# ChaissonLab/LRA

Measured on AMD Instinct MI355X. Metric: aligned Gbp/s, 30 kb ONT vs GRCh38 (MapRead_lowacc end to end incl. SAM text), per job, higher is better.
Workload: dtype int32

## Files before the change

### include/lra_hip.h

```cpp
#ifndef LRA_HIP_H_
#define LRA_HIP_H_
#include <stddef.h>
#include <stdint.h>

#ifdef __cplusplus
extern "C" {
#endif

typedef struct lra_ctx lra_ctx;

#define LRA_OK 0
#define LRA_ERR_INVALID (-1)
#define LRA_ERR_HIP (-2)
#define LRA_ERR_NOMEM (-3)

#define LRA_ST_OOB_SLOT 1
#define LRA_ST_NO_TERMINATION 2
#define LRA_ST_RANGE 4
#define LRA_ST_CAPACITY 8
#define LRA_ST_REJECTED 16
#define LRA_ST_UNSUPPORTED 32
#define LRA_ST_DEFERRED 64

int lra_ctx_create(int device_id, lra_ctx** out);
// ... 230 lines not shown
                           int mismatch, int indel, int max_freq, lra_refine_space_result* out);
int lra_refine_space_batch_mf(lra_ctx* ctx, int n, const char* d_qseq, const uint64_t* d_q_off, const int32_t* d_q_len, const char* d_tseq,
                              const uint64_t* d_t_off, const int32_t* d_t_len, const uint32_t* d_t_span, const int32_t* d_K, const int32_t* d_W,
                              const int32_t* d_diag, const uint32_t* d_q_add, const uint32_t* d_t_add, const uint32_t* d_flip_len, int match,
                              int mismatch, int indel, const int32_t* d_max_freq, lra_refine_space_result* out);

typedef struct lra_btwn_opts { int32_t K, W, refineSpaceDist; float anchorstoosparse; int32_t match, mismatch, indel, max_freq; } lra_btwn_opts;
typedef struct lra_btwn_result {
  uint64_t n_frags, n_matches, n_problems, n_pairs; uint32_t n_rounds;
  const uint64_t* d_match_off; const uint32_t* d_match_q; const uint32_t* d_match_t;
  const uint32_t* d_box; const float* d_eff; const uint8_t* d_refinespace;
} lra_btwn_result;
int lra_refine_btwn_splitchain_batch(lra_ctx* ctx, const lra_chain_result* chains, const lra_split_result* split, const lra_refined_result* refined,
                                     const uint64_t* d_read_off, const char* d_strands, uint64_t rc_base, const char* d_genome,
                                     const uint64_t* h_chrom_pos, int n_chrom, const lra_btwn_opts* opts, lra_btwn_result* out);

typedef struct lra_merge_result {
  uint64_t n_slots, n_groups, n_anchors;
  const uint64_t* d_slot_group_off;
  const uint64_t* d_cluster_base;
  const uint32_t* d_group_slot; const uint32_t* d_group_first; const uint32_t* d_group_last;
  const uint64_t* d_anchor_off;
  const uint32_t* d_count;
  const uint32_t* d_q; const uint32_t* d_t; const int32_t* d_len;
  const uint32_t* d_box; const int32_t* d_strand; const int32_t* d_chrom;
  const uint64_t* d_iota;
} lra_merge_result;
int lra_trim_anchor_pairs_batch(lra_ctx* ctx, uint64_t n_lists, const uint64_t* d_off, uint64_t n_anchors, uint32_t* d_q, uint32_t* d_t, int32_t* d_len);
int lra_trim_overlapped_anchors_batch(lra_ctx* ctx, uint64_t n_clusters, const uint64_t* d_off, uint64_t n_anchors, const int32_t* d_strand,
                                      uint32_t* d_q, uint32_t* d_t, int32_t* d_len);
// ... 437 lines not shown
```

### lra_amd/_lib.py

```python
import ctypes as C
import os

HERE = os.path.dirname(os.path.abspath(__file__))
_LIB = None
ABI_VERSION = 9


class LraError(RuntimeError):
    pass


def library_path():
    return os.path.join(HERE, "liblra_hip.so")


_u64p = C.POINTER(C.c_uint64)
_i32p = C.POINTER(C.c_int32)
_vp = C.c_void_p
SYMBOLS = {
    "lra_abi_version": (C.c_int, []),
    "lra_ctx_create": (C.c_int, [C.c_int, C.POINTER(_vp)]),
    "lra_ctx_destroy": (None, [_vp]),
    "lra_ctx_release_buffers": (C.c_int, [_vp, _u64p]),
    "lra_ctx_set_stream": (C.c_int, [_vp, _vp]),
# ... 73 lines not shown
    "lra_global_chain_batch": (C.c_int, [_vp, C.c_uint64, _vp, C.c_uint64, _vp, _vp, _vp, _vp, _vp, _vp]),
    "lra_split_chains_highacc_batch": (C.c_int, [_vp, C.c_uint64, _vp, C.c_uint64, _vp, _vp, _vp, _vp, _vp, C.c_int, _vp]),
    "lra_split_chains_batch": (C.c_int, [_vp, _vp, _vp, C.c_int, C.c_int, C.c_int, _vp]),
    "lra_format_sam": (C.c_int, [_vp, C.c_int, C.c_int, C.c_int, C.c_char_p, _vp, C.c_uint64, _vp]),
    "lra_format_sam_simple": (C.c_int, [_vp, C.c_int, C.c_char_p, _vp, C.c_uint64, _vp]),
    "lra_format_paf": (C.c_int, [_vp, C.c_int, _vp, C.c_uint64, _vp]),
    "lra_format_bed": (C.c_int, [_vp, _vp, C.c_uint64, _vp]),
    "lra_refine_space_batch": (C.c_int, [_vp, C.c_int] + [_vp] * 13 + [C.c_int] * 4 + [_vp]),
    "lra_refine_space_batch_mf": (C.c_int, [_vp, C.c_int] + [_vp] * 13 + [C.c_int] * 3 + [_vp, _vp]),
    "lra_between_anchors_batch": (C.c_int, [_vp, C.c_int] + [_vp] * 8 + [C.c_int] * 5 + [_vp]),
    "lra_refine_breakpoint_batch": (C.c_int, [_vp, C.c_int] + [_vp] * 16),
    "lra_sparse_dp_boxes_batch": (C.c_int, [_vp, C.c_int, _vp, _vp, _vp, _vp, _vp, _vp, _vp, _vp, _vp, _vp, _vp, _vp]),
    "lra_split_clusters_batch": (C.c_int, [_vp, C.c_int, _vp, _vp, _vp, _vp, _vp, _vp, _vp, _vp, _vp, C.c_int, C.c_int, _vp]),
    "lra_refine_splitchain_batch": (C.c_int, [_vp, _vp, _vp, _vp, _vp, C.c_int, _vp, C.c_uint64, _vp, _vp, _vp, _vp, _vp]),
    "lra_refine_btwn_splitchain_batch": (C.c_int, [_vp, _vp, _vp, _vp, _vp, _vp, C.c_uint64, _vp, _vp, C.c_int, _vp, _vp]),
    "lra_trim_anchor_pairs_batch": (C.c_int, [_vp, C.c_uint64, _vp, C.c_uint64, _vp, _vp, _vp]),
    "lra_merge_extend_batch": (C.c_int, [_vp, _vp, _vp, _vp, _vp, _vp, _vp, _vp, C.c_int, C.c_int, _vp]),
    "lra_format_sam_header": (C.c_int, [C.c_char_p, C.c_char_p, _vp, _vp, C.c_int, _vp, C.c_uint64, _vp]),
    "lra_alignment_strings": (C.c_int, [C.c_char_p, C.c_char_p, _vp, C.c_int, _vp, _vp, _vp, C.c_uint64, _vp, _vp]),
    "lra_md_string": (C.c_int, [C.c_char_p, C.c_char_p, C.c_uint64, _vp, C.c_uint64, _vp]),
    "lra_format_pairwise": (C.c_int, [C.c_char_p, C.c_char_p, C.c_int, C.c_int, C.c_int, C.c_uint32, C.c_char_p, C.c_char_p, C.c_char_p, C.c_uint64, _vp,
                                      C.c_uint64, _vp]),
    "lra_group_alignments": (C.c_int, [_vp, _vp, C.c_int, _vp]),
    "lra_order_alignments": (C.c_int, [_vp, C.c_int, _vp, _vp, C.c_int]),
    "lra_simple_mapqv": (C.c_int, [_vp, _vp, C.c_int, _vp, C.c_int, C.c_int, C.c_int, C.c_int]),
    "lra_output_read": (C.c_int, [_vp, _vp, C.c_int, _vp, C.c_int, C.c_char, C.c_int, C.c_char_p, C.c_int, _vp, _vp, C.c_uint64, _vp]),
    "lra_refine_clusters_batch": (C.c_int, [_vp, C.c_int] + [_vp] * 10 + [C.c_uint64, _vp, _vp, C.c_int, _vp, C.c_uint64, _vp, _vp, _vp, _vp, _vp]),
    "lra_local_refine_highacc_batch": (C.c_int, [_vp, C.c_uint64, _vp, _vp, _vp, _vp, C.c_uint64, _vp, _vp, _vp, _vp, _vp, _vp, C.c_uint64, _vp, _vp, _vp, _vp, _vp, C.c_uint64,
                                                 _vp, _vp, C.c_int, _vp, _vp]),
    "lra_local_refine_batch": (C.c_int, [_vp, C.c_uint64, _vp, _vp, _vp, C.c_uint64, _vp, _vp, _vp, _vp, _vp, _vp, C.c_uint64, _vp, _vp, _vp, _vp, _vp, C.c_uint64, _vp, _vp,
# ... 81 lines not shown
```

### lra_amd/chain.py

```python
import ctypes as C

import numpy as np

from .context import Context, ptr


class SdpOpts(C.Structure):
    _fields_ = [("rate", C.c_float), ("NumAln", C.c_int32), ("alnthres", C.c_float), ("gapopen", C.c_float), ("gapextend", C.c_float),
                ("gaproot", C.c_float), ("gapCeiling1", C.c_int32), ("gapCeiling2", C.c_int32), ("mode", C.c_int32),
                ("globalK", C.c_int32)]


ONT = dict(rate=20.0, NumAln=2, alnthres=0.65, gapopen=7.0, gapextend=10.0, gaproot=1.5, gapCeiling1=1500, gapCeiling2=3000, mode=0, globalK=17)


def sdp_opts(**kw):
    d = dict(ONT); d.update(kw)
    return SdpOpts(d["rate"], d["NumAln"], d["alnthres"], d["gapopen"], d["gapextend"], d["gaproot"], d["gapCeiling1"], d["gapCeiling2"], d["mode"],
                   d["globalK"])


class ChainResult(C.Structure):
    _fields_ = [("n_reads", C.c_int32), ("num_aln", C.c_int32), ("n_frags", C.c_uint64), ("n_points", C.c_uint64),
                ("n_subproblem_entries", C.c_uint64), ("d_n_chains", C.c_void_p), ("d_chain_start", C.c_void_p), ("d_chain_len", C.c_void_p),
# ... 136 lines not shown
    _fields_ = [("n_frags", C.c_uint64), ("n_matches", C.c_uint64), ("n_problems", C.c_uint64), ("n_pairs", C.c_uint64), ("n_rounds", C.c_uint32)] + [
        (n, C.c_void_p) for n in ("d_match_off", "d_match_q", "d_match_t", "d_box", "d_eff", "d_refinespace")]


def refine_btwn_splitchain_batch(ctx: Context, chains: ChainResult, split: SplitResult, refined: RefinedResult, read_off, strands, rc_base, genome,
                                 chrom_pos, K=10, W=5, refineSpaceDist=10000, anchorstoosparse=0.01, match=4, mismatch=-1, indel=-2, max_freq=15):
    cp = np.ascontiguousarray(chrom_pos, dtype=np.uint64)
    o = BtwnOpts(int(K), int(W), int(refineSpaceDist), float(anchorstoosparse), int(match), int(mismatch), int(indel), int(max_freq))
    res = BtwnResult()
    ctx.check(ctx.lib.lra_refine_btwn_splitchain_batch(ctx.h, C.byref(chains), C.byref(split), C.byref(refined), ptr(read_off), ptr(strands),
                                                       C.c_uint64(int(rc_base)), ptr(genome), C.c_void_p(cp.ctypes.data), len(cp) - 1, C.byref(o),
                                                       C.byref(res)))
    return res


def fetch_btwn(ctx: Context, res: BtwnResult):
    nf = res.n_frags
    return {"match_off": ctx.to_host(res.d_match_off, nf + 1, np.uint64), "match_q": ctx.to_host(res.d_match_q, res.n_matches, np.uint32),
            "match_t": ctx.to_host(res.d_match_t, res.n_matches, np.uint32), "box": ctx.to_host(res.d_box, 4 * nf, np.uint32).reshape(-1, 4),
            "eff": ctx.to_host(res.d_eff, nf, np.float32), "refinespace": ctx.to_host(res.d_refinespace, nf, np.uint8)}


class MergeResult(C.Structure):
    _fields_ = [("n_slots", C.c_uint64), ("n_groups", C.c_uint64), ("n_anchors", C.c_uint64)] + [(n, C.c_void_p) for n in (
        "d_slot_group_off", "d_cluster_base", "d_group_slot", "d_group_first", "d_group_last", "d_anchor_off", "d_count", "d_q", "d_t", "d_len", "d_box",
        "d_strand", "d_chrom", "d_iota")]


def merge_extend_batch(ctx: Context, chains: ChainResult, split: SplitResult, refined: BtwnResult, seq, read_off, genome, chrom_pos, K=10):
    cp = np.ascontiguousarray(chrom_pos, dtype=np.uint64)
# ... 174 lines not shown
```

### lra_amd/csrc/common.h

```cpp
#pragma once
#include <hip/hip_runtime.h>
#include <stdint.h>
#include <stdio.h>
#include <atomic>
#include <memory>
#include <string>
#include <string.h>
#include <vector>
#include "../../include/lra_hip.h"

struct lra_seed_state;
struct lra_cluster_state;
struct lra_map_state;
struct lra_handover;
void lra_handover_free(lra_ctx* ctx);
struct lra_gen_cell { std::atomic<uint64_t> gen{0}; std::atomic<bool> dead{false}; };
struct lra_time_rec { const char* name; hipEvent_t a, b; hipStream_t stream; };

struct lra_ctx {
  int device = 0;
  hipStream_t stream = nullptr;
  std::string err;
  void* scratch[4] = {nullptr, nullptr, nullptr, nullptr};
  size_t scratch_bytes[4] = {0, 0, 0, 0};
// ... 18 lines not shown
  void* gbuf[192] = {};
  size_t gbytes[192] = {};
  bool sdp_inner = false;
  bool sort_short = false;
  const char* sort_tag = "sort"; const char* sort_fb_tag = "sort_fallback";
  bool timing = false;
  std::vector<lra_time_rec> recs;
  std::vector<hipEvent_t> free_events;
  lra_ctx* child = nullptr;
  bool owns_stream = false;
  bool pipelined = false;
  struct lra_handover* handover = nullptr;
  struct { bool valid = false; int n_reads = 0; const char* d_seq = nullptr; const uint64_t* d_read_off = nullptr; int k = 0, w = 0, max_freq = 0; lra_seed_result res; } ahead;
  bool store_all = false;
  int svsig_len = 25;
  bool low_priority = false; int prio = 0;
};

hipStream_t lra_side_fork(lra_ctx* ctx, int i = 0);
void lra_side_join(lra_ctx* ctx, int i = 0);
hipError_t lra_segsort_pairs(lra_ctx* ctx, void* temp, size_t& temp_bytes, const uint64_t* kin, uint64_t* kout, const uint32_t* vin, uint32_t* vout, unsigned int total,
                             unsigned int nseg, const uint64_t* b, const uint64_t* e, int begin_bit, int end_bit, hipStream_t st);
void lra_time_begin(lra_ctx* ctx, const char* name, hipStream_t stream = nullptr);
void lra_time_end(lra_ctx* ctx, hipStream_t stream = nullptr);
void lra_seed_free(lra_ctx* ctx);
void lra_cluster_free(lra_ctx* ctx);
void lra_map_free(lra_ctx* ctx);

int lra_set_err(lra_ctx* ctx, int code, const char* fmt, ...);
int lra_host_threads();
// ... 27 lines not shown
```

### lra_amd/csrc/refine_btwn.hip

```cpp
#include "common.h"
#include "scan.h"
#include <rocprim/rocprim.hpp>
#include <algorithm>
#include <vector>

namespace {

constexpr uint32_t NONE = 0xFFFFFFFFu;

struct Seg { uint64_t off; uint32_t len; uint32_t next; };

struct BtArgs {
  uint64_t n_slots; int numAln;
  const uint32_t* nChains; const uint64_t* chainStart; const uint32_t* nSplit; const uint32_t* spStatus; const uint8_t* spStrand; const int32_t* spChrom;
  const uint8_t* splitLink;
  const uint64_t* read_off; uint64_t rcBase;
  const uint64_t* pos; int npos;
  int K, W; uint32_t RSD; float sparse2;
  int round;
  uint32_t* box; uint32_t* cnt; uint8_t* rspace; uint32_t* segHead; uint32_t* segTail;
  uint32_t* need; const uint64_t* needOff;
  uint64_t* pQoff; int32_t* pQlen; uint64_t* pToff; int32_t* pTlen; uint32_t* pTspan; int32_t* pK; int32_t* pW; int32_t* pDiag; uint32_t* pQadd;
  uint32_t* pTadd; uint32_t* pFlip;
  uint32_t* mSpan; uint8_t* mKind; uint8_t* mTwo; uint8_t* mSt; uint32_t* mX; uint32_t* mXp;
  const uint64_t* pairOff; const uint64_t* pool; uint64_t poolU, poolS;
  Seg* segs; uint32_t* segCount; uint32_t segCap; uint32_t* overflow;
};

__device__ __forceinline__ int space_diag(uint32_t qe, uint32_t qs) {
  return min((int)floorf(fmaxf(100.f, 0.15f * (float)(qe - qs))), 1000);
}

__device__ void plan_problem(const BtArgs& a, uint64_t s, int j, uint64_t r, uint32_t readLen, int chrom, uint32_t qe, uint32_t qs, uint32_t te, uint32_t ts,
                             int st, uint32_t lrts, uint32_t lrlength, int kind, int two, uint32_t x, uint32_t xp) {
  if (st == 1) { const uint32_t t = qs; qs = readLen - qe; qe = readLen - t; }
  const uint64_t i = 2 * s + j;
  a.need[i] = 1;
  a.pQoff[i] = (st ? a.rcBase : 0) + a.read_off[r] + qs; a.pQlen[i] = (int32_t)(qe - qs);
  a.pToff[i] = a.pos[chrom] + (ts - lrts); a.pTlen[i] = (int32_t)(te - ts + lrlength); a.pTspan[i] = te - (ts - lrts);
  a.pK[i] = a.K; a.pW[i] = a.W; a.pDiag[i] = space_diag(qe, qs); a.pQadd[i] = qs; a.pTadd[i] = ts - lrts; a.pFlip[i] = st == 1 ? readLen : 0;
  a.mSpan[i] = min(qe - qs, te - ts); a.mKind[i] = (uint8_t)kind; a.mTwo[i] = (uint8_t)two; a.mSt[i] = (uint8_t)st; a.mX[i] = x; a.mXp[i] = xp;
}

__global__ void bt_plan(BtArgs a) {
  const uint64_t s = (uint64_t)blockIdx.x * blockDim.x + threadIdx.x;
  if (s >= a.n_slots) return;
  a.need[2 * s] = 0; a.need[2 * s + 1] = 0;
  const uint64_t r = s / a.numAln;
  if ((uint32_t)(s % a.numAln) >= a.nChains[r] || a.spStatus[s]) return;
  const uint32_t nsp = a.nSplit[s];
  const uint64_t cs = a.chainStart[s];
  const uint32_t readLen = (uint32_t)(a.read_off[r + 1] - a.read_off[r]);
  auto glen = [&](int c) { return a.pos[c + 1] - a.pos[c]; };
  if (a.round >= 1) {
    const uint32_t c = (uint32_t)a.round;
    if (c >= nsp) return;
    const uint64_t xc = cs + c, xp = cs + c - 1;
    if (a.cnt[xc] == 0 || a.cnt[xp] == 0) return;
    const uint32_t cqs = a.box[4 * xc], cqe = a.box[4 * xc + 1], cts = a.box[4 * xc + 2], cte = a.box[4 * xc + 3];
    const uint32_t pqs = a.box[4 * xp], pts = a.box[4 * xp + 2], pte = a.box[4 * xp + 3];
    (void)cqs;
    const int cst = a.spStrand[xc], pst = a.spStrand[xp], link = a.splitLink[cs + c - 1];
    const int cchrom = a.spChrom[xc], pchrom = a.spChrom[xp];
    const uint32_t qs = cqe, qe = pqs;
    uint32_t ts1 = 0, te1 = 0, ts2 = 0, te2 = 0;
    if (qe <= qs) return;
    const uint32_t gap = qe - qs;
    int st1 = 0, st2 = 0, two = 0;
    if (cst == pst && link == 0) {
      two = 0; st1 = cst;
      if (cte <= pts) { ts1 = cte; te1 = pts; }
      else if (cts > pte) { ts1 = pte; te1 = cts; }
      else return;
    } else if (cst != pst && link == 1) {
      st1 = cst; st2 = pst; two = 1;
      if (cte <= pts) {
// ... 2 lines not shown
      } else if (cts > pte) {
        if (st1 == 0) { ts1 = cte; te1 = ts1 + gap; te2 = cts; ts2 = te2 > gap ? te2 - gap : 0; }
        else { te1 = cts; ts1 = te1 > gap ? te1 - gap : 0; te2 = pts; ts2 = te2 > gap ? te2 - gap : 0; }
      } else return;
    } else if (cst == pst && link == 1) {
      st1 = cst; st2 = st1; two = 1;
      if (st1 == 0 && cte > pts) { ts1 = cte; te1 = ts1 + gap; te2 = pts; ts2 = te2 > gap ? te2 - gap : 0; }
      else if (st1 == 1 && cts < pte) { te1 = cts; ts1 = te1 > gap ? te1 - gap : 0; ts2 = pte; te2 = ts2 + gap; }
      else return;
    }
    if (te1 <= ts1) return;
    if (te1 >= glen(cchrom)) return;
    if (max(gap, te1 - ts1) >= 5 * a.RSD) return;
    uint32_t space = max(gap, te1 - ts1);
    if (space >= 20 && space <= a.RSD && cchrom == pchrom)
      plan_problem(a, s, 0, r, readLen, cchrom, qe, qs, te1, ts1, st1, 0, 0, 0, two, (uint32_t)(xc - cs), (uint32_t)(xp - cs));
    if (two) {
      if (te2 <= ts2) return;
      if (te2 >= glen(cchrom)) return;
      if (max(gap, te2 - ts2) >= 5 * a.RSD) return;
      space = max(gap, te2 - ts2);
      if (space >= 20 && space <= a.RSD && cchrom == pchrom)
        plan_problem(a, s, 1, r, readLen, pchrom, qe, qs, te2, ts2, st2, 0, 0, 1, 1, (uint32_t)(xp - cs), (uint32_t)(xp - cs));
    }
    return;
  }
  if (nsp == 0) return;
  if (a.round == -1) {
    const uint64_t x = cs;
    if (a.cnt[x] == 0) return;
    const int st = a.spStrand[x], chrom = a.spChrom[x];
    const uint32_t qs = a.box[4 * x + 1], qe = readLen;
    uint32_t ts = 0, te = 0;
    if (st == 0) { ts = a.box[4 * x + 3]; te = ts + qe - qs; }
    else { te = a.box[4 * x + 2]; if (te > qe - qs) ts = te - (qe - qs); else return; }
    if (!(qe > qs && te > ts)) return;
    const uint32_t space = max(qe - qs, te - ts);
    if (!(space >= 20 && space < a.RSD && (uint64_t)te + 500 < glen(chrom))) return;
    uint32_t lrts = 0, lrlength = 0;
    if (st == 0) { lrts = 0; lrlength = 500; } else { if (ts > 500) lrts = 500; lrlength = lrts; }
    plan_problem(a, s, 0, r, readLen, chrom, qe, qs, te, ts, st, lrts, lrlength, 1, 1, 0, 0);
  } else {
    const uint64_t x = cs + nsp - 1;
    if (a.cnt[x] == 0) return;
    const int st = a.spStrand[x], chrom = a.spChrom[x];
    const uint32_t qs = 0, qe = a.box[4 * x];
    uint32_t ts, te;
    if (st == 0) { te = a.box[4 * x + 2]; ts = te > qe - qs ? te - (qe - qs) : 0; }
    else { ts = a.box[4 * x + 3]; te = ts + (qe - qs); }
    if (!(qe > qs && te > ts)) return;
    const uint32_t space = max(qe - qs, te - ts);
    if (!(space >= 20 && space < a.RSD && (uint64_t)te + 500 < glen(chrom))) return;
    uint32_t lrts = 0, lrlength = 0;
    if (st == 0) { if (ts > 500) lrts = 500; lrlength = lrts; } else { lrts = 0; lrlength = 500; }
    plan_problem(a, s, 0, r, readLen, chrom, qe, qs, te, ts, st, lrts, lrlength, 1, 1, nsp - 1, nsp - 1);
  }
}

__global__ void bt_compact(BtArgs a, uint64_t* dQoff, int32_t* dQlen, uint64_t* dToff, int32_t* dTlen, uint32_t* dTspan, int32_t* dK, int32_t* dW,
                           int32_t* dDiag, uint32_t* dQadd, uint32_t* dTadd, uint32_t* dFlip) {
  const uint64_t i = (uint64_t)blockIdx.x * blockDim.x + threadIdx.x;
  if (i >= 2 * a.n_slots || !a.need[i]) return;
  const uint64_t p = a.needOff[i];
  dQoff[p] = a.pQoff[i]; dQlen[p] = a.pQlen[i]; dToff[p] = a.pToff[i]; dTlen[p] = a.pTlen[i]; dTspan[p] = a.pTspan[i]; dK[p] = a.pK[i]; dW[p] = a.pW[i];
  dDiag[p] = a.pDiag[i]; dQadd[p] = a.pQadd[i]; dTadd[p] = a.pTadd[i]; dFlip[p] = a.pFlip[i];
}

__global__ void bt_pack(uint64_t n, const uint32_t* __restrict__ q, const uint32_t* __restrict__ t, uint64_t* out) {
  const uint64_t i = (uint64_t)blockIdx.x * blockDim.x + threadIdx.x;
  if (i < n) out[i] = ((uint64_t)q[i] << 32) | t[i];
}

__device__ void append_seg(const BtArgs& a, uint64_t x, uint64_t off, uint32_t len) {
  if (len == 0) return;
  const uint32_t id = atomicAdd(a.segCount, 1u);
  if (id >= a.segCap) { *a.overflow = 1; return; }
  a.segs[id].off = off; a.segs[id].len = len; a.segs[id].next = NONE;
  if (a.segHead[x] == NONE) a.segHead[x] = id; else a.segs[a.segTail[x]].next = id;
  a.segTail[x] = id;
  uint32_t qs = a.box[4 * x], qe = a.box[4 * x + 1], ts = a.box[4 * x + 2], te = a.box[4 * x + 3];
  for (uint32_t i = 0; i < len; i++) {
    const uint64_t v = a.pool[off + i];
    const uint32_t q = (uint32_t)(v >> 32), t = (uint32_t)v;
    qs = min(qs, q); qe = max(qe, q + (uint32_t)a.K); ts = min(ts, t); te = max(te, t + (uint32_t)a.K);
  }
  a.box[4 * x] = qs; a.box[4 * x + 1] = qe; a.box[4 * x + 2] = ts; a.box[4 * x + 3] = te;
  a.cnt[x] += len;
}

__global__ void bt_apply(BtArgs a) {
  const uint64_t s = (uint64_t)blockIdx.x * blockDim.x + threadIdx.x;
  if (s >= a.n_slots) return;
  for (int j = 0; j < 2; j++) {
    const uint64_t i = 2 * s + j;
    if (!a.need[i]) continue;
    const uint64_t cs = a.chainStart[s];
    const uint64_t p = a.needOff[i];
    const uint64_t p0 = a.pairOff[p];
    const uint32_t n = (uint32_t)(a.pairOff[p + 1] - p0);
    const float eff = ((float)n) / (float)a.mSpan[i];
    const uint64_t x = cs + a.mX[i], xp = cs + a.mXp[i];
    if (n == 0) continue;
    if (a.mKind[i] == 1) { append_seg(a, x, a.poolU + p0, n); a.rspace[x] = 1; continue; }
    if (eff >= a.sparse2) { append_seg(a, x, a.poolU + p0, n); a.rspace[x] = 1; continue; }
    if (a.mTwo[i]) continue;
    const uint64_t* S = a.pool + a.poolS + p0;
    const int st = a.mSt[i];
    uint32_t start = 0;
    while (start < n) {
      uint32_t end = start + 1;
      while (end < n) {
        const long long dq = llabs((long long)(uint32_t)(S[end] >> 32) - (long long)(uint32_t)(S[end - 1] >> 32));
        const long long dt = llabs((long long)(uint32_t)S[end] - (long long)(uint32_t)S[end - 1]);
        if (min(dq, dt) <= 200) end++; else break;
      }
      if (end - start >= 4) {
// ... 3 lines not shown
          tE = max(tE, t + (uint32_t)a.K); tS = min(tS, t); qE = max(qE, q + (uint32_t)a.K); qS = min(qS, q);
        }
        const uint32_t cqe = a.box[4 * x + 1], cts = a.box[4 * x + 2], cte = a.box[4 * x + 3];
        const uint32_t pqs = a.box[4 * xp], pts = a.box[4 * xp + 2], pte = a.box[4 * xp + 3];
        int qd = qS >= cqe ? (int)(qS - cqe) : 0, td;
        if (st == 0) td = tS >= cte ? (int)(tS - cte) : 0; else td = cts >= tE ? (int)(cts - tE) : 0;
        const int dist_cur = max(qd, td);
        qd = pqs >= qE ? (int)(pqs - qE) : 0;
        if (st == 0) td = pts >= tE ? (int)(pts - tE) : 0; else td = tS >= pte ? (int)(tS - pte) : 0;
        const int dist_prev = max(qd, td);
        append_seg(a, dist_cur <= dist_prev ? x : xp, a.poolS + p0 + start, end - start);
      }
      start = end;
    }
  }
}

struct LayArgs {
  uint64_t n_slots; int numAln; int K;
  const uint32_t* nChains; const uint64_t* chainStart; const uint32_t* nSplit; const uint32_t* spStatus;
  const uint64_t* baseOff; const uint32_t* baseQ; const uint32_t* baseT;
  const uint32_t* cnt; const uint32_t* box; const uint32_t* segHead; const Seg* segs; const uint64_t* pool;
  const uint64_t* outOff; uint32_t* oq; uint32_t* ot; float* eff;
};

__global__ void __launch_bounds__(64) bt_layout(LayArgs a) {
  const uint64_t s = blockIdx.x;
  const uint64_t r = s / a.numAln;
  if ((uint32_t)(s % a.numAln) >= a.nChains[r] || a.spStatus[s]) return;
  const uint64_t cs = a.chainStart[s];
// ... 41 lines not shown
  ctx->gbuf[slot] = p; ctx->gbytes[slot] = want;
  return p;
}

}

extern "C" int lra_refine_btwn_splitchain_batch(lra_ctx* ctx, const lra_chain_result* ch, const lra_split_result* sp, const lra_refined_result* rf,
                                                const uint64_t* d_read_off, const char* d_strands, uint64_t rc_base, const char* d_genome,
                                                const uint64_t* h_chrom_pos, int n_chrom, const lra_btwn_opts* opts, lra_btwn_result* out) {
  if (!ctx || !ch || !sp || !rf || !out || !opts || !h_chrom_pos || n_chrom < 1) return LRA_ERR_INVALID;
  memset(out, 0, sizeof *out);
  LRA_HIP_CHECK(ctx, hipSetDevice(ctx->device));
  hipStream_t st = ctx->stream;
  const uint64_t slots = sp->n_slots, NF = sp->n_frags;
  out->n_frags = NF;
  if (slots == 0) return LRA_OK;
  const size_t npos = (size_t)n_chrom + 1, n2 = 2 * slots;
  auto take = [](char*& p, size_t n, size_t e) { char* r = p; p += sz(n, e); return r; };
  char* w = (char*)lra_ensure(ctx, 35, sz(NF + 2, 4) * 3 + sz(4 * NF + 4, 4) + sz(NF + 2, 1) + sz(NF + 2, 8) + sz(NF + 1, 4) + sz(npos, 8) + sz(n2 + 1, 4) * 12 +
                                           sz(n2 + 2, 8) * 3 + sz(n2 + 1, 1) * 3 + 4096);
  if (!w) return LRA_ERR_NOMEM;
  BtArgs a;
  memset(&a, 0, sizeof a);
  a.n_slots = slots; a.numAln = ch->num_aln; a.nChains = ch->d_n_chains; a.chainStart = ch->d_chain_start; a.nSplit = sp->d_n_split; a.spStatus = sp->d_status;
  a.spStrand = sp->d_sp_strand; a.spChrom = sp->d_sp_chrom; a.splitLink = sp->d_split_link; a.read_off = d_read_off; a.rcBase = rc_base;
  a.K = opts->K; a.W = opts->W; a.RSD = (uint32_t)opts->refineSpaceDist; a.sparse2 = opts->anchorstoosparse * 2;
  a.cnt = (uint32_t*)take(w, NF + 2, 4); a.segHead = (uint32_t*)take(w, NF + 2, 4); a.segTail = (uint32_t*)take(w, NF + 2, 4);
  a.box = (uint32_t*)take(w, 4 * NF + 4, 4); a.rspace = (uint8_t*)take(w, NF + 2, 1);
  uint64_t* outOff = (uint64_t*)take(w, NF + 2, 8); float* eff = (float*)take(w, NF + 1, 4);
  uint64_t* dpos = (uint64_t*)take(w, npos, 8);
  a.pos = dpos; a.npos = (int)npos;
  a.need = (uint32_t*)take(w, n2 + 1, 4); a.pQlen = (int32_t*)take(w, n2 + 1, 4); a.pTlen = (int32_t*)take(w, n2 + 1, 4); a.pTspan = (uint32_t*)take(w, n2 + 1, 4);
  a.pK = (int32_t*)take(w, n2 + 1, 4); a.pW = (int32_t*)take(w, n2 + 1, 4); a.pDiag = (int32_t*)take(w, n2 + 1, 4); a.pQadd = (uint32_t*)take(w, n2 + 1, 4);
  a.pTadd = (uint32_t*)take(w, n2 + 1, 4); a.pFlip = (uint32_t*)take(w, n2 + 1, 4); a.mSpan = (uint32_t*)take(w, n2 + 1, 4); a.mX = (uint32_t*)take(w, n2 + 1, 4);
  uint64_t* needOff = (uint64_t*)take(w, n2 + 2, 8); a.pQoff = (uint64_t*)take(w, n2 + 2, 8); a.pToff = (uint64_t*)take(w, n2 + 2, 8);
  a.mKind = (uint8_t*)take(w, n2 + 1, 1); a.mTwo = (uint8_t*)take(w, n2 + 1, 1); a.mSt = (uint8_t*)take(w, n2 + 1, 1);
  a.needOff = needOff;
  char* wd = (char*)lra_ensure(ctx, 36, sz(n2 + 1, 4) * 10 + sz(n2 + 1, 8) * 2 + 4096);
  if (!wd) return LRA_ERR_NOMEM;
  a.mXp = (uint32_t*)take(wd, n2 + 1, 4);
  uint64_t* dQoff = (uint64_t*)take(wd, n2 + 1, 8); uint64_t* dToff = (uint64_t*)take(wd, n2 + 1, 8);
  int32_t* dQlen = (int32_t*)take(wd, n2 + 1, 4); int32_t* dTlen = (int32_t*)take(wd, n2 + 1, 4); uint32_t* dTspan = (uint32_t*)take(wd, n2 + 1, 4);
  int32_t* dK = (int32_t*)take(wd, n2 + 1, 4); int32_t* dW = (int32_t*)take(wd, n2 + 1, 4); int32_t* dDiag = (int32_t*)take(wd, n2 + 1, 4);
  uint32_t* dQadd = (uint32_t*)take(wd, n2 + 1, 4); uint32_t* dTadd = (uint32_t*)take(wd, n2 + 1, 4); uint32_t* dFlip = (uint32_t*)take(wd, n2 + 1, 4);
  LRA_HIP_CHECK(ctx, hipMemcpyAsync(dpos, h_chrom_pos, npos * 8, hipMemcpyHostToDevice, st));
  hipLaunchKernelGGL(bt_init, dim3((unsigned)((NF + 256) / 256)), dim3(256), 0, st, NF, rf->d_match_off, rf->d_box, a.cnt, a.box, a.segHead, a.segTail, a.rspace);
  std::vector<uint32_t> h_nsplit(slots);
  LRA_HIP_CHECK(ctx, hipMemcpyAsync(h_nsplit.data(), sp->d_n_split, slots * 4, hipMemcpyDeviceToHost, st));
  LRA_HIP_CHECK(ctx, hipStreamSynchronize(st));
  uint32_t maxSplit = 0;
  for (uint64_t i = 0; i < slots; i++) maxSplit = std::max(maxSplit, h_nsplit[i]);
  const int SEG_SLOT = 32, POOL_SLOT = 33, OUT_SLOT = 34;
  uint32_t* segCtl = (uint32_t*)lra_scratch(ctx, 3, 256);
  if (!segCtl) return LRA_ERR_NOMEM;
  LRA_HIP_CHECK(ctx, hipMemsetAsync(segCtl, 0, 256, st));
  a.segCount = segCtl; a.overflow = segCtl + 1;
  uint64_t poolUsed = 0; uint32_t segUsedBound = 0;
  std::vector<int> rounds;
  for (uint32_t c = 1; c < maxSplit; c++) rounds.push_back((int)c);
  if (maxSplit > 0) { rounds.push_back(-1); rounds.push_back(-2); }
  const unsigned gs = (unsigned)((slots + 255) / 256), g2 = (unsigned)((n2 + 255) / 256);
  uint64_t totalProblems = 0, totalPairs = 0;
  for (int rd : rounds) {
    a.round = rd;
    lra_time_begin(ctx, "btwn_plan");
    hipLaunchKernelGGL(bt_plan, dim3(gs), dim3(256), 0, st, a);
    lra_time_end(ctx);
    { int rc = lra_exclusive_scan<uint32_t>(ctx, (long)n2, a.need, needOff); if (rc) return rc; }
    uint64_t np = 0;
    LRA_HIP_CHECK(ctx, hipMemcpyAsync(&np, needOff + n2, 8, hipMemcpyDeviceToHost, st));
    LRA_HIP_CHECK(ctx, hipStreamSynchronize(st));
    if (np == 0) continue;
    totalProblems += np;
    hipLaunchKernelGGL(bt_compact, dim3(g2), dim3(256), 0, st, a, dQoff, dQlen, dToff, dTlen, dTspan, dK, dW, dDiag, dQadd, dTadd, dFlip);
    lra_refine_space_result rs;
    { int rc = lra_refine_space_batch(ctx, (int)np, d_strands, dQoff, dQlen, d_genome, dToff, dTlen, dTspan, dK, dW, dDiag, dQadd, dTadd, dFlip, opts->match,
                                      opts->mismatch, opts->indel, opts->max_freq, &rs); if (rc) return rc; }
    const uint64_t nP = rs.n_pairs;
    totalPairs += nP;
    uint64_t* pool = (uint64_t*)grow_keep(ctx, POOL_SLOT, poolUsed * 8, (poolUsed + 2 * nP + 2) * 8);
    if (!pool) return LRA_ERR_NOMEM;
    const uint32_t segPrev = segUsedBound;
    segUsedBound += (uint32_t)(nP / 4 + 2 * np + 2);
    Seg* segs = (Seg*)grow_keep(ctx, SEG_SLOT, (size_t)segPrev * sizeof(Seg), (size_t)segUsedBound * sizeof(Seg));
    if (!segs) return LRA_ERR_NOMEM;
    a.pool = pool; a.poolU = poolUsed; a.poolS = poolUsed + nP; a.segs = segs; a.segCap = segUsedBound; a.pairOff = rs.d_pair_off;
    if (nP > 0) {
      lra_time_begin(ctx, "btwn_apply");
      hipLaunchKernelGGL(bt_pack, dim3((unsigned)((nP + 255) / 256)), dim3(256), 0, st, nP, rs.d_pair_q, rs.d_pair_t, pool + poolUsed);
      size_t temp_bytes = 0;
      (void)rocprim::segmented_radix_sort_keys(nullptr, temp_bytes, (uint64_t*)nullptr, (uint64_t*)nullptr, (unsigned int)nP, (unsigned int)np, (uint64_t*)nullptr,
                                               (uint64_t*)nullptr, 0, 64, st);
      void* temp = lra_scratch(ctx, 2, temp_bytes + 256);
      if (!temp) { lra_time_end(ctx); return LRA_ERR_NOMEM; }
      hipError_t e = rocprim::segmented_radix_sort_keys(temp, temp_bytes, pool + poolUsed, pool + poolUsed + nP, (unsigned int)nP, (unsigned int)np, rs.d_pair_off,
                                                        rs.d_pair_off + 1, 0, 64, st);
      lra_time_end(ctx);
      if (e != hipSuccess) return lra_set_err(ctx, LRA_ERR_HIP, "segmented sort: %s", hipGetErrorString(e));
    }
    lra_time_begin(ctx, "btwn_apply");
    hipLaunchKernelGGL(bt_apply, dim3(gs), dim3(256), 0, st, a);
    lra_time_end(ctx);
    poolUsed += 2 * nP;
  }
  uint32_t ctl[2] = {0, 0};
  LRA_HIP_CHECK(ctx, hipMemcpyAsync(ctl, segCtl, 8, hipMemcpyDeviceToHost, st));
  LRA_HIP_CHECK(ctx, hipStreamSynchronize(st));
  if (ctl[1]) return lra_set_err(ctx, LRA_ERR_HIP, "internal: segment pool overflow");
  { int rc = lra_exclusive_scan<uint32_t>(ctx, (long)NF + 1, a.cnt, outOff); if (rc) return rc; }
  uint64_t NM = 0;
  LRA_HIP_CHECK(ctx, hipMemcpyAsync(&NM, outOff + NF, 8, hipMemcpyDeviceToHost, st));
  LRA_HIP_CHECK(ctx, hipStreamSynchronize(st));
  char* wm = (char*)lra_ensure(ctx, OUT_SLOT, sz(NM + 1, 4) * 2 + 1024);
  if (!wm) return LRA_ERR_NOMEM;
  uint32_t* oq = (uint32_t*)take(wm, NM + 1, 4); uint32_t* ot = (uint32_t*)take(wm, NM + 1, 4);
  LayArgs l;
  memset(&l, 0, sizeof l);
  l.n_slots = slots; l.numAln = ch->num_aln; l.K = opts->K; l.nChains = ch->d_n_chains; l.chainStart = ch->d_chain_start; l.nSplit = sp->d_n_split; l.spStatus = sp->d_status;
  l.baseOff = rf->d_match_off; l.baseQ = rf->d_match_q; l.baseT = rf->d_match_t; l.cnt = a.cnt; l.box = a.box; l.segHead = a.segHead;
  l.segs = (const Seg*)ctx->gbuf[SEG_SLOT]; l.pool = (const uint64_t*)ctx->gbuf[POOL_SLOT]; l.outOff = outOff; l.oq = oq; l.ot = ot; l.eff = eff;
  lra_time_begin(ctx, "btwn_apply");
  hipLaunchKernelGGL(bt_layout, dim3((unsigned)slots), dim3(64), 0, st, l);
  lra_time_end(ctx);
  LRA_HIP_CHECK(ctx, hipStreamSynchronize(st));
  LRA_HIP_CHECK(ctx, hipGetLastError());
  out->n_matches = NM; out->n_problems = totalProblems; out->n_pairs = totalPairs; out->n_rounds = (uint32_t)rounds.size();
  out->d_match_off = outOff; out->d_match_q = oq; out->d_match_t = ot; out->d_box = a.box; out->d_eff = eff; out->d_refinespace = a.rspace;
  return LRA_OK;
}
```

Measured before the change: 1.085.

## Plan all chain gaps speculatively per pass and verify-apply sequentially

Replaces the fixed per-round loop (one gap per chain per round, maxSplit+1 rounds) with a speculative scheme. Each pass plans every remaining gap of every unfinished chain at once, solves them in one refine-space batch, and then applies them in order per slot. Application stops at the first gap whose re-planned problem differs from the speculative one, and later passes redo the rejected gaps. This is meant to collapse many small rounds, each with host syncs and launches, into a few large passes. The cost is larger planning buffers and wasted refine work on rejected speculative problems.

After: 1.070. 1.4% lower.

```diff
diff --git a/include/lra_hip.h b/include/lra_hip.h
--- a/include/lra_hip.h
+++ b/include/lra_hip.h
@@ -268,6 +268,7 @@
 int lra_refine_btwn_splitchain_batch(lra_ctx* ctx, const lra_chain_result* chains, const lra_split_result* split, const lra_refined_result* refined,
                                      const uint64_t* d_read_off, const char* d_strands, uint64_t rc_base, const char* d_genome,
                                      const uint64_t* h_chrom_pos, int n_chrom, const lra_btwn_opts* opts, lra_btwn_result* out);
+int lra_refine_btwn_splitchain_stats(lra_ctx* ctx, uint64_t* passes, uint64_t* accepted, uint64_t* rejected);
 
 typedef struct lra_merge_result {
   uint64_t n_slots, n_groups, n_anchors;
diff --git a/lra_amd/_lib.py b/lra_amd/_lib.py
--- a/lra_amd/_lib.py
+++ b/lra_amd/_lib.py
@@ -111,6 +111,7 @@
     "lra_split_clusters_batch": (C.c_int, [_vp, C.c_int, _vp, _vp, _vp, _vp, _vp, _vp, _vp, _vp, _vp, C.c_int, C.c_int, _vp]),
     "lra_refine_splitchain_batch": (C.c_int, [_vp, _vp, _vp, _vp, _vp, C.c_int, _vp, C.c_uint64, _vp, _vp, _vp, _vp, _vp]),
     "lra_refine_btwn_splitchain_batch": (C.c_int, [_vp, _vp, _vp, _vp, _vp, _vp, C.c_uint64, _vp, _vp, C.c_int, _vp, _vp]),
+    "lra_refine_btwn_splitchain_stats": (C.c_int, [_vp, _vp, _vp, _vp]),
     "lra_trim_anchor_pairs_batch": (C.c_int, [_vp, C.c_uint64, _vp, C.c_uint64, _vp, _vp, _vp]),
     "lra_merge_extend_batch": (C.c_int, [_vp, _vp, _vp, _vp, _vp, _vp, _vp, _vp, C.c_int, C.c_int, _vp]),
     "lra_format_sam_header": (C.c_int, [C.c_char_p, C.c_char_p, _vp, _vp, C.c_int, _vp, C.c_uint64, _vp]),
diff --git a/lra_amd/chain.py b/lra_amd/chain.py
--- a/lra_amd/chain.py
+++ b/lra_amd/chain.py
@@ -174,6 +174,12 @@
     return res
 
 
+def refine_btwn_splitchain_stats(ctx: Context):
+    v = (C.c_uint64 * 3)()
+    ctx.check(ctx.lib.lra_refine_btwn_splitchain_stats(ctx.h, C.byref(v, 0), C.byref(v, 8), C.byref(v, 16)))
+    return {"passes": int(v[0]), "accepted": int(v[1]), "rejected": int(v[2])}
+
+
 def fetch_btwn(ctx: Context, res: BtwnResult):
     nf = res.n_frags
     return {"match_off": ctx.to_host(res.d_match_off, nf + 1, np.uint64), "match_q": ctx.to_host(res.d_match_q, res.n_matches, np.uint32),
diff --git a/lra_amd/csrc/common.h b/lra_amd/csrc/common.h
--- a/lra_amd/csrc/common.h
+++ b/lra_amd/csrc/common.h
@@ -56,6 +56,7 @@
   struct { bool valid = false; int n_reads = 0; const char* d_seq = nullptr; const uint64_t* d_read_off = nullptr; int k = 0, w = 0, max_freq = 0; lra_seed_result res; } ahead;
   bool store_all = false;
   int svsig_len = 25;
+  uint64_t btwn_passes = 0, btwn_accepted = 0, btwn_rejected = 0;
   bool low_priority = false; int prio = 0;
 };
 
diff --git a/lra_amd/csrc/refine_btwn.hip b/lra_amd/csrc/refine_btwn.hip
--- a/lra_amd/csrc/refine_btwn.hip
+++ b/lra_amd/csrc/refine_btwn.hip
@@ -17,49 +17,51 @@
   const uint64_t* read_off; uint64_t rcBase;
   const uint64_t* pos; int npos;
   int K, W; uint32_t RSD; float sparse2;
-  int round;
   uint32_t* box; uint32_t* cnt; uint8_t* rspace; uint32_t* segHead; uint32_t* segTail;
+  uint32_t* spos; uint32_t* rem; const uint64_t* itemOff; uint64_t itemCap;
   uint32_t* need; const uint64_t* needOff;
   uint64_t* pQoff; int32_t* pQlen; uint64_t* pToff; int32_t* pTlen; uint32_t* pTspan; int32_t* pK; int32_t* pW; int32_t* pDiag; uint32_t* pQadd;
   uint32_t* pTadd; uint32_t* pFlip;
   uint32_t* mSpan; uint8_t* mKind; uint8_t* mTwo; uint8_t* mSt; uint32_t* mX; uint32_t* mXp;
   const uint64_t* pairOff; const uint64_t* pool; uint64_t poolU, poolS;
   Seg* segs; uint32_t* segCount; uint32_t segCap; uint32_t* overflow;
+  unsigned long long* stat;
 };
 
 __device__ __forceinline__ int space_diag(uint32_t qe, uint32_t qs) {
   return min((int)floorf(fmaxf(100.f, 0.15f * (float)(qe - qs))), 1000);
 }
 
-__device__ void plan_problem(const BtArgs& a, uint64_t s, int j, uint64_t r, uint32_t readLen, int chrom, uint32_t qe, uint32_t qs, uint32_t te, uint32_t ts,
+struct Prob {
+  uint64_t qoff, toff; int32_t qlen, tlen, k, w, diag; uint32_t tspan, qadd, tadd, flip, span, x, xp; uint8_t kind, two, st;
+};
+struct GapPlan { uint32_t need[2]; Prob p[2]; };
+
+__device__ void plan_problem(const BtArgs& a, GapPlan& g, int j, uint64_t r, uint32_t readLen, int chrom, uint32_t qe, uint32_t qs, uint32_t te, uint32_t ts,
                              int st, uint32_t lrts, uint32_t lrlength, int kind, int two, uint32_t x, uint32_t xp) {
   if (st == 1) { const uint32_t t = qs; qs = readLen - qe; qe = readLen - t; }
-  const uint64_t i = 2 * s + j;
-  a.need[i] = 1;
-  a.pQoff[i] = (st ? a.rcBase : 0) + a.read_off[r] + qs; a.pQlen[i] = (int32_t)(qe - qs);
-  a.pToff[i] = a.pos[chrom] + (ts - lrts); a.pTlen[i] = (int32_t)(te - ts + lrlength); a.pTspan[i] = te - (ts - lrts);
-  a.pK[i] = a.K; a.pW[i] = a.W; a.pDiag[i] = space_diag(qe, qs); a.pQadd[i] = qs; a.pTadd[i] = ts - lrts; a.pFlip[i] = st == 1 ? readLen : 0;
-  a.mSpan[i] = min(qe - qs, te - ts); a.mKind[i] = (uint8_t)kind; a.mTwo[i] = (uint8_t)two; a.mSt[i] = (uint8_t)st; a.mX[i] = x; a.mXp[i] = xp;
-}
-
-__global__ void bt_plan(BtArgs a) {
-  const uint64_t s = (uint64_t)blockIdx.x * blockDim.x + threadIdx.x;
-  if (s >= a.n_slots) return;
-  a.need[2 * s] = 0; a.need[2 * s + 1] = 0;
+  Prob& p = g.p[j];
+  g.need[j] = 1;
+  p.qoff = (st ? a.rcBase : 0) + a.read_off[r] + qs; p.qlen = (int32_t)(qe - qs);
+  p.toff = a.pos[chrom] + (ts - lrts); p.tlen = (int32_t)(te - ts + lrlength); p.tspan = te - (ts - lrts);
+  p.k = a.K; p.w = a.W; p.diag = space_diag(qe, qs); p.qadd = qs; p.tadd = ts - lrts; p.flip = st == 1 ? readLen : 0;
+  p.span = min(qe - qs, te - ts); p.kind = (uint8_t)kind; p.two = (uint8_t)two; p.st = (uint8_t)st; p.x = x; p.xp = xp;
+}
+
+__device__ void plan_gap(const BtArgs& a, uint64_t s, int round, GapPlan& g) {
+  g.need[0] = 0; g.need[1] = 0;
   const uint64_t r = s / a.numAln;
-  if ((uint32_t)(s % a.numAln) >= a.nChains[r] || a.spStatus[s]) return;
   const uint32_t nsp = a.nSplit[s];
   const uint64_t cs = a.chainStart[s];
   const uint32_t readLen = (uint32_t)(a.read_off[r + 1] - a.read_off[r]);
   auto glen = [&](int c) { return a.pos[c + 1] - a.pos[c]; };
-  if (a.round >= 1) {
-    const uint32_t c = (uint32_t)a.round;
+  if (round >= 1) {
+    const uint32_t c = (uint32_t)round;
     if (c >= nsp) return;
     const uint64_t xc = cs + c, xp = cs + c - 1;
     if (a.cnt[xc] == 0 || a.cnt[xp] == 0) return;
-    const uint32_t cqs = a.box[4 * xc], cqe = a.box[4 * xc + 1], cts = a.box[4 * xc + 2], cte = a.box[4 * xc + 3];
+    const uint32_t cqe = a.box[4 * xc + 1], cts = a.box[4 * xc + 2], cte = a.box[4 * xc + 3];
     const uint32_t pqs = a.box[4 * xp], pts = a.box[4 * xp + 2], pte = a.box[4 * xp + 3];
-    (void)cqs;
     const int cst = a.spStrand[xc], pst = a.spStrand[xp], link = a.splitLink[cs + c - 1];
     const int cchrom = a.spChrom[xc], pchrom = a.spChrom[xp];
     const uint32_t qs = cqe, qe = pqs;
@@ -92,19 +94,19 @@
     if (max(gap, te1 - ts1) >= 5 * a.RSD) return;
     uint32_t space = max(gap, te1 - ts1);
     if (space >= 20 && space <= a.RSD && cchrom == pchrom)
-      plan_problem(a, s, 0, r, readLen, cchrom, qe, qs, te1, ts1, st1, 0, 0, 0, two, (uint32_t)(xc - cs), (uint32_t)(xp - cs));
+      plan_problem(a, g, 0, r, readLen, cchrom, qe, qs, te1, ts1, st1, 0, 0, 0, two, (uint32_t)(xc - cs), (uint32_t)(xp - cs));
     if (two) {
       if (te2 <= ts2) return;
       if (te2 >= glen(cchrom)) return;
       if (max(gap, te2 - ts2) >= 5 * a.RSD) return;
       space = max(gap, te2 - ts2);
       if (space >= 20 && space <= a.RSD && cchrom == pchrom)
-        plan_problem(a, s, 1, r, readLen, pchrom, qe, qs, te2, ts2, st2, 0, 0, 1, 1, (uint32_t)(xp - cs), (uint32_t)(xp - cs));
+        plan_problem(a, g, 1, r, readLen, pchrom, qe, qs, te2, ts2, st2, 0, 0, 1, 1, (uint32_t)(xp - cs), (uint32_t)(xp - cs));
     }
     return;
   }
   if (nsp == 0) return;
-  if (a.round == -1) {
+  if (round == -1) {
     const uint64_t x = cs;
     if (a.cnt[x] == 0) return;
     const int st = a.spStrand[x], chrom = a.spChrom[x];
@@ -117,7 +119,7 @@
     if (!(space >= 20 && space < a.RSD && (uint64_t)te + 500 < glen(chrom))) return;
     uint32_t lrts = 0, lrlength = 0;
     if (st == 0) { lrts = 0; lrlength = 500; } else { if (ts > 500) lrts = 500; lrlength = lrts; }
-    plan_problem(a, s, 0, r, readLen, chrom, qe, qs, te, ts, st, lrts, lrlength, 1, 1, 0, 0);
+    plan_problem(a, g, 0, r, readLen, chrom, qe, qs, te, ts, st, lrts, lrlength, 1, 1, 0, 0);
   } else {
     const uint64_t x = cs + nsp - 1;
     if (a.cnt[x] == 0) return;
@@ -131,14 +133,51 @@
     if (!(space >= 20 && space < a.RSD && (uint64_t)te + 500 < glen(chrom))) return;
     uint32_t lrts = 0, lrlength = 0;
     if (st == 0) { if (ts > 500) lrts = 500; lrlength = lrts; } else { lrts = 0; lrlength = 500; }
-    plan_problem(a, s, 0, r, readLen, chrom, qe, qs, te, ts, st, lrts, lrlength, 1, 1, nsp - 1, nsp - 1);
-  }
+    plan_problem(a, g, 0, r, readLen, chrom, qe, qs, te, ts, st, lrts, lrlength, 1, 1, nsp - 1, nsp - 1);
+  }
+}
+
+__device__ __forceinline__ int gap_round(uint32_t p, uint32_t nsp) { return p + 1 < nsp ? (int)(p + 1) : (p + 1 == nsp ? -1 : -2); }
+
+__global__ void bt_init_slots(BtArgs a) {
+  const uint64_t s = (uint64_t)blockIdx.x * blockDim.x + threadIdx.x;
+  if (s >= a.n_slots) return;
+  const uint64_t r = s / a.numAln;
+  const bool live = (uint32_t)(s % a.numAln) < a.nChains[r] && !a.spStatus[s] && a.nSplit[s] > 0;
+  a.spos[s] = 0; a.rem[s] = live ? a.nSplit[s] + 1 : 0;
+}
+
+__global__ void bt_plan(BtArgs a) {
+  const uint64_t it = (uint64_t)blockIdx.x * blockDim.x + threadIdx.x;
+  if (it >= a.itemCap) return;
+  a.need[2 * it] = 0; a.need[2 * it + 1] = 0;
+  if (it >= a.itemOff[a.n_slots]) return;
+  uint64_t lo = 0, hi = a.n_slots;
+  while (hi - lo > 1) { const uint64_t mid = (lo + hi) / 2; if (a.itemOff[mid] <= it) lo = mid; else hi = mid; }
+  const uint64_t s = lo;
+  GapPlan g;
+  plan_gap(a, s, gap_round(a.spos[s] + (uint32_t)(it - a.itemOff[s]), a.nSplit[s]), g);
+  for (int j = 0; j < 2; j++) {
+    if (!g.need[j]) continue;
+    const uint64_t i = 2 * it + j;
+    const Prob& p = g.p[j];
+    a.need[i] = 1;
+    a.pQoff[i] = p.qoff; a.pQlen[i] = p.qlen; a.pToff[i] = p.toff; a.pTlen[i] = p.tlen; a.pTspan[i] = p.tspan; a.pK[i] = p.k; a.pW[i] = p.w; a.pDiag[i] = p.diag;
+    a.pQadd[i] = p.qadd; a.pTadd[i] = p.tadd; a.pFlip[i] = p.flip;
+    a.mSpan[i] = p.span; a.mKind[i] = p.kind; a.mTwo[i] = p.two; a.mSt[i] = p.st; a.mX[i] = p.x; a.mXp[i] = p.xp;
+  }
+}
+
+__device__ __forceinline__ bool same_problem(const BtArgs& a, uint64_t i, const Prob& p) {
+  return a.pQoff[i] == p.qoff && a.pQlen[i] == p.qlen && a.pToff[i] == p.toff && a.pTlen[i] == p.tlen && a.pTspan[i] == p.tspan && a.pK[i] == p.k && a.pW[i] == p.w &&
+         a.pDiag[i] == p.diag && a.pQadd[i] == p.qadd && a.pTadd[i] == p.tadd && a.pFlip[i] == p.flip && a.mSpan[i] == p.span && a.mKind[i] == p.kind &&
+         a.mTwo[i] == p.two && a.mSt[i] == p.st && a.mX[i] == p.x && a.mXp[i] == p.xp;
 }
 
 __global__ void bt_compact(BtArgs a, uint64_t* dQoff, int32_t* dQlen, uint64_t* dToff, int32_t* dTlen, uint32_t* dTspan, int32_t* dK, int32_t* dW,
                            int32_t* dDiag, uint32_t* dQadd, uint32_t* dTadd, uint32_t* dFlip) {
   const uint64_t i = (uint64_t)blockIdx.x * blockDim.x + threadIdx.x;
-  if (i >= 2 * a.n_slots || !a.need[i]) return;
+  if (i >= 2 * a.itemCap || !a.need[i]) return;
   const uint64_t p = a.needOff[i];
   dQoff[p] = a.pQoff[i]; dQlen[p] = a.pQlen[i]; dToff[p] = a.pToff[i]; dTlen[p] = a.pTlen[i]; dTspan[p] = a.pTspan[i]; dK[p] = a.pK[i]; dW[p] = a.pW[i];
   dDiag[p] = a.pDiag[i]; dQadd[p] = a.pQadd[i]; dTadd[p] = a.pTadd[i]; dFlip[p] = a.pFlip[i];
@@ -166,11 +205,10 @@
   a.cnt[x] += len;
 }
 
-__global__ void bt_apply(BtArgs a) {
-  const uint64_t s = (uint64_t)blockIdx.x * blockDim.x + threadIdx.x;
-  if (s >= a.n_slots) return;
+__device__ uint64_t apply_gap(const BtArgs& a, uint64_t s, uint64_t it) {
+  uint64_t pairs = 0;
   for (int j = 0; j < 2; j++) {
-    const uint64_t i = 2 * s + j;
+    const uint64_t i = 2 * it + j;
     if (!a.need[i]) continue;
     const uint64_t cs = a.chainStart[s];
     const uint64_t p = a.needOff[i];
@@ -178,6 +216,7 @@
     const uint32_t n = (uint32_t)(a.pairOff[p + 1] - p0);
     const float eff = ((float)n) / (float)a.mSpan[i];
     const uint64_t x = cs + a.mX[i], xp = cs + a.mXp[i];
+    pairs += n;
     if (n == 0) continue;
     if (a.mKind[i] == 1) { append_seg(a, x, a.poolU + p0, n); a.rspace[x] = 1; continue; }
     if (eff >= a.sparse2) { append_seg(a, x, a.poolU + p0, n); a.rspace[x] = 1; continue; }
@@ -211,6 +250,33 @@
       start = end;
     }
   }
+  return pairs;
+}
+
+__global__ void bt_verify_apply(BtArgs a) {
+  const uint64_t s = (uint64_t)blockIdx.x * blockDim.x + threadIdx.x;
+  if (s >= a.n_slots) return;
+  const uint32_t R = a.rem[s];
+  if (R == 0) return;
+  const uint64_t base = a.itemOff[s];
+  const uint32_t p0 = a.spos[s], nsp = a.nSplit[s];
+  unsigned long long acc = 0, rej = 0, pairs = 0;
+  uint32_t k = 0;
+  for (; k < R; k++) {
+    const uint64_t it = base + k;
+    GapPlan g;
+    plan_gap(a, s, gap_round(p0 + k, nsp), g);
+    bool same = true;
+    for (int j = 0; j < 2; j++) same = same && a.need[2 * it + j] == g.need[j] && (!g.need[j] || same_problem(a, 2 * it + j, g.p[j]));
+    if (!same) break;
+    acc += g.need[0] + g.need[1];
+    pairs += apply_gap(a, s, it);
+  }
+  for (uint32_t d = k; d < R; d++) rej += a.need[2 * (base + d)] + a.need[2 * (base + d) + 1];
+  a.spos[s] = p0 + k; a.rem[s] = R - k;
+  if (acc) atomicAdd(a.stat, acc);
+  if (rej) atomicAdd(a.stat + 1, rej);
+  if (pairs) atomicAdd(a.stat + 2, pairs);
 }
 
 struct LayArgs {
@@ -282,11 +348,13 @@
   hipStream_t st = ctx->stream;
   const uint64_t slots = sp->n_slots, NF = sp->n_frags;
   out->n_frags = NF;
+  ctx->btwn_passes = 0; ctx->btwn_accepted = 0; ctx->btwn_rejected = 0;
   if (slots == 0) return LRA_OK;
-  const size_t npos = (size_t)n_chrom + 1, n2 = 2 * slots;
+  const uint64_t itemMax = NF + slots;
+  const size_t npos = (size_t)n_chrom + 1, n2 = 2 * itemMax;
   auto take = [](char*& p, size_t n, size_t e) { char* r = p; p += sz(n, e); return r; };
-  char* w = (char*)lra_ensure(ctx, 35, sz(NF + 2, 4) * 3 + sz(4 * NF + 4, 4) + sz(NF + 2, 1) + sz(NF + 2, 8) + sz(NF + 1, 4) + sz(npos, 8) + sz(n2 + 1, 4) * 12 +
-                                           sz(n2 + 2, 8) * 3 + sz(n2 + 1, 1) * 3 + 4096);
+  char* w = (char*)lra_ensure(ctx, 35, sz(NF + 2, 4) * 3 + sz(4 * NF + 4, 4) + sz(NF + 2, 1) + sz(NF + 2, 8) + sz(NF + 1, 4) + sz(npos, 8) + sz(slots + 1, 4) * 2 +
+                                           sz(slots + 2, 8) + sz(n2 + 1, 4) * 12 + sz(n2 + 2, 8) * 3 + sz(n2 + 1, 1) * 3 + 4096);
   if (!w) return LRA_ERR_NOMEM;
   BtArgs a;
   memset(&a, 0, sizeof a);
@@ -298,6 +366,9 @@
   uint64_t* outOff = (uint64_t*)take(w, NF + 2, 8); float* eff = (float*)take(w, NF + 1, 4);
   uint64_t* dpos = (uint64_t*)take(w, npos, 8);
   a.pos = dpos; a.npos = (int)npos;
+  a.spos = (uint32_t*)take(w, slots + 1, 4); a.rem = (uint32_t*)take(w, slots + 1, 4);
+  uint64_t* itemOff = (uint64_t*)take(w, slots + 2, 8);
+  a.itemOff = itemOff;
   a.need = (uint32_t*)take(w, n2 + 1, 4); a.pQlen = (int32_t*)take(w, n2 + 1, 4); a.pTlen = (int32_t*)take(w, n2 + 1, 4); a.pTspan = (uint32_t*)take(w, n2 + 1, 4);
   a.pK = (int32_t*)take(w, n2 + 1, 4); a.pW = (int32_t*)take(w, n2 + 1, 4); a.pDiag = (int32_t*)take(w, n2 + 1, 4); a.pQadd = (uint32_t*)take(w, n2 + 1, 4);
   a.pTadd = (uint32_t*)take(w, n2 + 1, 4); a.pFlip = (uint32_t*)take(w, n2 + 1, 4); a.mSpan = (uint32_t*)take(w, n2 + 1, 4); a.mX = (uint32_t*)take(w, n2 + 1, 4);
@@ -313,39 +384,44 @@
   uint32_t* dQadd = (uint32_t*)take(wd, n2 + 1, 4); uint32_t* dTadd = (uint32_t*)take(wd, n2 + 1, 4); uint32_t* dFlip = (uint32_t*)take(wd, n2 + 1, 4);
   LRA_HIP_CHECK(ctx, hipMemcpyAsync(dpos, h_chrom_pos, npos * 8, hipMemcpyHostToDevice, st));
   hipLaunchKernelGGL(bt_init, dim3((unsigned)((NF + 256) / 256)), dim3(256), 0, st, NF, rf->d_match_off, rf->d_box, a.cnt, a.box, a.segHead, a.segTail, a.rspace);
+  const unsigned gs = (unsigned)((slots + 255) / 256);
+  hipLaunchKernelGGL(bt_init_slots, dim3(gs), dim3(256), 0, st, a);
   std::vector<uint32_t> h_nsplit(slots);
   LRA_HIP_CHECK(ctx, hipMemcpyAsync(h_nsplit.data(), sp->d_n_split, slots * 4, hipMemcpyDeviceToHost, st));
   LRA_HIP_CHECK(ctx, hipStreamSynchronize(st));
   uint32_t maxSplit = 0;
   for (uint64_t i = 0; i < slots; i++) maxSplit = std::max(maxSplit, h_nsplit[i]);
+  const uint32_t nRounds = maxSplit > 0 ? maxSplit - 1 + 2 : 0;
   const int SEG_SLOT = 32, POOL_SLOT = 33, OUT_SLOT = 34;
   uint32_t* segCtl = (uint32_t*)lra_scratch(ctx, 3, 256);
   if (!segCtl) return LRA_ERR_NOMEM;
   LRA_HIP_CHECK(ctx, hipMemsetAsync(segCtl, 0, 256, st));
-  a.segCount = segCtl; a.overflow = segCtl + 1;
+  a.segCount = segCtl; a.overflow = segCtl + 1; a.stat = (unsigned long long*)(segCtl + 2);
   uint64_t poolUsed = 0; uint32_t segUsedBound = 0;
-  std::vector<int> rounds;
-  for (uint32_t c = 1; c < maxSplit; c++) rounds.push_back((int)c);
-  if (maxSplit > 0) { rounds.push_back(-1); rounds.push_back(-2); }
-  const unsigned gs = (unsigned)((slots + 255) / 256), g2 = (unsigned)((n2 + 255) / 256);
-  uint64_t totalProblems = 0, totalPairs = 0;
-  for (int rd : rounds) {
-    a.round = rd;
+  uint64_t itemCap = itemMax;
+  uint32_t passes = 0;
+  const bool dbg = getenv("LRA_BTWN_DBG") != nullptr;
+  for (;;) {
+    { int rc = lra_exclusive_scan<uint32_t>(ctx, (long)slots, a.rem, itemOff); if (rc) return rc; }
+    a.itemCap = itemCap;
     lra_time_begin(ctx, "btwn_plan");
-    hipLaunchKernelGGL(bt_plan, dim3(gs), dim3(256), 0, st, a);
+    hipLaunchKernelGGL(bt_plan, dim3((unsigned)((itemCap + 255) / 256)), dim3(256), 0, st, a);
     lra_time_end(ctx);
-    { int rc = lra_exclusive_scan<uint32_t>(ctx, (long)n2, a.need, needOff); if (rc) return rc; }
-    uint64_t np = 0;
-    LRA_HIP_CHECK(ctx, hipMemcpyAsync(&np, needOff + n2, 8, hipMemcpyDeviceToHost, st));
+    { int rc = lra_exclusive_scan<uint32_t>(ctx, (long)(2 * itemCap), a.need, needOff); if (rc) return rc; }
+    uint64_t nItems = 0, np = 0;
+    LRA_HIP_CHECK(ctx, hipMemcpyAsync(&nItems, itemOff + slots, 8, hipMemcpyDeviceToHost, st));
+    LRA_HIP_CHECK(ctx, hipMemcpyAsync(&np, needOff + 2 * itemCap, 8, hipMemcpyDeviceToHost, st));
     LRA_HIP_CHECK(ctx, hipStreamSynchronize(st));
-    if (np == 0) continue;
-    totalProblems += np;
-    hipLaunchKernelGGL(bt_compact, dim3(g2), dim3(256), 0, st, a, dQoff, dQlen, dToff, dTlen, dTspan, dK, dW, dDiag, dQadd, dTadd, dFlip);
+    if (nItems == 0) break;
+    passes++;
+    if (dbg) fprintf(stderr, "[btwn] pass %u: %llu gaps of unfinished chains, %llu problems\n", passes, (unsigned long long)nItems, (unsigned long long)np);
+    if (np == 0) break;
+    hipLaunchKernelGGL(bt_compact, dim3((unsigned)((2 * itemCap + 255) / 256)), dim3(256), 0, st, a, dQoff, dQlen, dToff, dTlen, dTspan, dK, dW, dDiag, dQadd,
+                       dTadd, dFlip);
     lra_refine_space_result rs;
     { int rc = lra_refine_space_batch(ctx, (int)np, d_strands, dQoff, dQlen, d_genome, dToff, dTlen, dTspan, dK, dW, dDiag, dQadd, dTadd, dFlip, opts->match,
                                       opts->mismatch, opts->indel, opts->max_freq, &rs); if (rc) return rc; }
     const uint64_t nP = rs.n_pairs;
-    totalPairs += nP;
     uint64_t* pool = (uint64_t*)grow_keep(ctx, POOL_SLOT, poolUsed * 8, (poolUsed + 2 * nP + 2) * 8);
     if (!pool) return LRA_ERR_NOMEM;
     const uint32_t segPrev = segUsedBound;
@@ -367,12 +443,13 @@
       if (e != hipSuccess) return lra_set_err(ctx, LRA_ERR_HIP, "segmented sort: %s", hipGetErrorString(e));
     }
     lra_time_begin(ctx, "btwn_apply");
-    hipLaunchKernelGGL(bt_apply, dim3(gs), dim3(256), 0, st, a);
+    hipLaunchKernelGGL(bt_verify_apply, dim3(gs), dim3(256), 0, st, a);
     lra_time_end(ctx);
     poolUsed += 2 * nP;
-  }
-  uint32_t ctl[2] = {0, 0};
-  LRA_HIP_CHECK(ctx, hipMemcpyAsync(ctl, segCtl, 8, hipMemcpyDeviceToHost, st));
+    itemCap = nItems;
+  }
+  uint32_t ctl[8] = {};
+  LRA_HIP_CHECK(ctx, hipMemcpyAsync(ctl, segCtl, sizeof ctl, hipMemcpyDeviceToHost, st));
   LRA_HIP_CHECK(ctx, hipStreamSynchronize(st));
   if (ctl[1]) return lra_set_err(ctx, LRA_ERR_HIP, "internal: segment pool overflow");
   { int rc = lra_exclusive_scan<uint32_t>(ctx, (long)NF + 1, a.cnt, outOff); if (rc) return rc; }
@@ -392,7 +469,20 @@
   lra_time_end(ctx);
   LRA_HIP_CHECK(ctx, hipStreamSynchronize(st));
   LRA_HIP_CHECK(ctx, hipGetLastError());
-  out->n_matches = NM; out->n_problems = totalProblems; out->n_pairs = totalPairs; out->n_rounds = (uint32_t)rounds.size();
+  uint64_t stat[3];
+  memcpy(stat, ctl + 2, sizeof stat);
+  ctx->btwn_passes = passes; ctx->btwn_accepted = stat[0]; ctx->btwn_rejected = stat[1];
+  if (dbg) fprintf(stderr, "[btwn] %u passes, %llu problems accepted, %llu rejected, %llu pairs\n", passes, (unsigned long long)stat[0], (unsigned long long)stat[1],
+                   (unsigned long long)stat[2]);
+  out->n_matches = NM; out->n_problems = stat[0]; out->n_pairs = stat[2]; out->n_rounds = nRounds;
   out->d_match_off = outOff; out->d_match_q = oq; out->d_match_t = ot; out->d_box = a.box; out->d_eff = eff; out->d_refinespace = a.rspace;
   return LRA_OK;
 }
+
+extern "C" int lra_refine_btwn_splitchain_stats(lra_ctx* ctx, uint64_t* passes, uint64_t* accepted, uint64_t* rejected) {
+  if (!ctx) return LRA_ERR_INVALID;
+  if (passes) *passes = ctx->btwn_passes;
+  if (accepted) *accepted = ctx->btwn_accepted;
+  if (rejected) *rejected = ctx->btwn_rejected;
+  return LRA_OK;
+}
```
